# brendel-group/cl-ica

Hardware: AMD Instinct MI355X
Metric: training steps/sec (B=6144, n=10 MLP) (higher is better)
Workload: dtype f32 via f16x2 split (3 fp16 MFMA products of scaled two-piece operands, fp32 accumulate)

## Files before the change

cl_ica_amd/csrc/lp_finalize.h:

```cpp
#pragma once
#include "lp_kernels.h"

namespace clica {
namespace lp {

__device__ __forceinline__ float pos_sum(const float* a, const float* b, int n, const Params& q, bool frac) {
  float s = 0.f;
  for (int k = 0; k < n; ++k) {
    float d = a[k] - b[k];
    float t;
    if (frac) t = fexp2(q.p * flog2(fabsf(d) + 1e-12f));
    else if (q.p == 2.f) t = d * d;
    else if (q.p == 1.f) t = fabsf(d);
    else if (q.p == 3.f) t = fabsf(d) * d * d;
    else t = fabsf(d) > 0.f ? fexp2(q.p * flog2(fabsf(d))) : 0.f;
    s += t;
  }
  return s;
}


__device__ __forceinline__ float unfused(float t) { asm("" : "+v"(t)); return t; }
typedef const __attribute__((address_space(3))) float* lds_cfloat_ptr;
template <int W>
// ... 75 lines not shown
  const float sc = q.xs * C / tau;
  statC[i] = sc;
  if (statC_value) *statC_value = sc;
  if (!dz1 && !dz2) return;
  if (dot) {
    float pos = 0.f;
    if (q.posdot) pos = q.posdot[i];
    else for (int k = 0; k < q.n; ++k) pos += a[k] * b[k];
    const float dpos = -A / tau + (C / tau) * fexp2(pos * q.kscale - L2);
    if (q.dpos) { q.dpos[i] = dpos; return; }
    for (int k = 0; k < q.n; ++k) {
      if (dz1) dz1[i * ldd1 + k] = dpos * b[k];
      if (dz2) dz2[i * ldd2 + k] = dpos * a[k];
    }
    return;
  }
  const float sp_ = pos_sum(a, b, q.n, q, frac != 0);
  const float cpos = cpos_of(sp_, A, C, q, tau, compat, L2);
  for (int k = 0; k < q.n; ++k) {
    const float d = a[k] - b[k];
    float dt;
    if (frac) {
      const float v = fexp2((q.p - 1.f) * flog2(fabsf(d) + 1e-12f));
      dt = d > 0.f ? v : (d < 0.f ? -v : 0.f);
    } else if (q.p == 2.f) dt = d;
    else if (q.p == 1.f) dt = (d > 0.f ? 1.f : 0.f) - (d < 0.f ? 1.f : 0.f);
    else if (q.p == 3.f) dt = d * fabsf(d);
    else {
      const float ad = fabsf(d);
      const float v = ad > 0.f ? fexp2((q.p - 1.f) * flog2(ad)) : 0.f;
      dt = d < 0.f ? -v : v;
    }
    const float g = cpos * dt;
    if (dz1) dz1[i * ldd1 + k] = g;
    if (dz2) dz2[i * ldd2 + k] = -g;
  }
}

template <int W>
__device__ __forceinline__ void coef_row_regs(
    const int64_t i, const int64_t rows, const float (&a)[W], const float (&b)[W], const float sp_,
    const Params& q, float tau, float alpha, int compat, const float L2,
    float* __restrict__ statL, float* __restrict__ statC,
    float* __restrict__ dz1, int64_t ldd1, float* __restrict__ dz2, int64_t ldd2, float* statC_value) {
  const float inv_rows = 1.f / (float)rows;
  const float gi = 1.f * inv_rows + 0.f;
  const float A = 2.f * alpha * gi + 0.f;
  const float C = 2.f * (1.f - alpha) * gi + 0.f;
  statL[i] = L2;
  const float sc = q.xs * C / tau;
  statC[i] = sc;
  *statC_value = sc;
  if (!dz1 && !dz2) return;
  const float cpos = cpos_of(sp_, A, C, q, tau, compat, L2);
  const int n = q.n;
  auto put = [&](int k, float dt) {
    const float g = cpos * dt;
    if (k < n) {
      if (dz1) dz1[i * ldd1 + k] = g;
      if (dz2) dz2[i * ldd2 + k] = -g;
    }
  };
  if (q.p == 2.f) {
#pragma unroll
    for (int k = 0; k < W; ++k) { const float d = a[k] - b[k]; put(k, d); }
  } else if (q.p == 1.f) {
#pragma unroll
    for (int k = 0; k < W; ++k) { const float d = a[k] - b[k]; put(k, (d > 0.f ? 1.f : 0.f) - (d < 0.f ? 1.f : 0.f)); }
  } else if (q.p == 3.f) {
#pragma unroll
    for (int k = 0; k < W; ++k) { const float d = a[k] - b[k]; put(k, d * fabsf(d)); }
  } else {
#pragma unroll
    for (int k = 0; k < W; ++k) {
      const float d = a[k] - b[k];
      const float ad = fabsf(d);
      const float v = ad > 0.f ? fexp2((q.p - 1.f) * flog2(ad)) : 0.f;
      put(k, d < 0.f ? -v : v);
    }
  }
}


struct FinScratch { float* sm; float* ss; float* zr0; float* zr1; int zmaxn; float* ush; };
template <bool COHERENT = false, int W = 0>
__device__ __forceinline__ void finalize_rows(
    const int blk, const float2* __restrict__ part, const int nsplit, const int64_t rows,
    const float* __restrict__ z1, int64_t ld1, const float* __restrict__ z2, int64_t ld2,
    const Params& q, float tau, float alpha, int compat, int frac, int dot, float log_b3,
    float* __restrict__ loss_i, float* __restrict__ pos_i, float* __restrict__ lse_i, const TrainOut& T, const FinScratch& S,
    float& v_loss, float& v_pos, float& v_lse) {
  const int lane_row = threadIdx.x & (FIN_ROWS - 1), grp = threadIdx.x / FIN_ROWS;
  const int64_t i = (int64_t)blk * FIN_ROWS + lane_row;
  const bool staged = q.n <= S.zmaxn;
  if (staged) {
    const int64_t r0 = (int64_t)blk * FIN_ROWS;
    const int cnt = (int)min((int64_t)FIN_ROWS, rows - r0) * q.n;
    for (int idx = threadIdx.x; idx < cnt; idx += THREADS) {
      const int r = idx / q.n, k = idx - r * q.n;
      S.zr0[idx] = z1[(r0 + r) * ld1 + k];
      S.zr1[idx] = z2[(r0 + r) * ld2 + k];
    }
  }
  float m = -1e30f, s = 0.f;
  if (i < rows) {
    constexpr int G = THREADS / FIN_ROWS;
    for (int sp0 = grp; sp0 < nsplit; sp0 += 4 * G) {
      float2 ps[4];
#pragma unroll
      for (int u = 0; u < 4; ++u) {
        const int sp = sp0 + u * G;
        if (!(sp < nsplit)) ps[u] = make_float2(-1e30f, 0.f);
        else if (COHERENT)
          ps[u] = __builtin_bit_cast(float2, __hip_atomic_load(reinterpret_cast<const unsigned long long*>(part + (int64_t)sp * rows + i),
                                                                __ATOMIC_RELAXED, __HIP_MEMORY_SCOPE_AGENT));
        else ps[u] = part[(int64_t)sp * rows + i];
      }
#pragma unroll
      for (int u = 0; u < 4; ++u) {
        const float mn = fmaxf(m, ps[u].x);
        s = s * fexp2(m - mn) + ps[u].y * fexp2(ps[u].x - mn);
        m = mn;
      }
    }
  }
  S.sm[grp * FIN_ROWS + lane_row] = m; S.ss[grp * FIN_ROWS + lane_row] = s;
  __syncthreads();
  v_loss = 0.f; v_pos = 0.f; v_lse = 0.f;
  if (grp == 0 && i < rows) {
#pragma unroll
    for (int w = 1; w < THREADS / FIN_ROWS; ++w) {
      const float pm = S.sm[w * FIN_ROWS + lane_row], psum = S.ss[w * FIN_ROWS + lane_row];
      const float mn = fmaxf(m, pm);
      s = s * fexp2(m - mn) + psum * fexp2(pm - mn);
      m = mn;
    }
    float pos, xp;
    const float* ra = staged ? &S.zr0[lane_row * q.n] : z1 + i * ld1;
    const float* rb = staged ? &S.zr1[lane_row * q.n] : z2 + i * ld2;
    const bool regs = W > 0 && staged && !dot && !frac;
    float av[W > 0 ? W : 1], bv[W > 0 ? W : 1], sp_regs = 0.f;
    if constexpr (W > 0) {
      if (regs) { read_staged_row<W>(av, &S.zr0[lane_row * q.n], q.n); read_staged_row<W>(bv, &S.zr1[lane_row * q.n], q.n); }
    }
    if (dot) {
      pos = 0.f;
      if (q.posdot) pos = q.posdot[i];
      else for (int k = 0; k < q.n; ++k) pos += ra[k] * rb[k];
      xp = pos * q.kscale;
      pos = -pos;
    } else {
      float sp_;
      if constexpr (W > 0) sp_ = regs ? pos_sum_regs<W>(av, bv, q.n, q) : pos_sum(ra, rb, q.n, q, frac != 0);
      else sp_ = pos_sum(ra, rb, q.n, q, frac != 0);
      sp_regs = sp_;
      pos = q.pow ? sp_ : root_of<true>(sp_, q);
      xp = -pos * q.kscale;
    }
    if (compat) {
      const float mn = fmaxf(m, xp);
      s = s * fexp2(m - mn) + fexp2(xp - mn);
      m = mn;
    }
    const float L2 = m + flog2(s);
    const float lse_raw = L2 * kLn2;
    const float lse = compat ? lse_raw : lse_raw - log_b3;
    const float lp = pos / tau;
    const float li = 2.f * (alpha * lp + (1.f - alpha) * lse);
    loss_i[i] = li; pos_i[i] = lp; lse_i[i] = L2;
    float sc_i = 0.f;
    if (T.statL) {
      bool done = false;
      if constexpr (W > 0) {
        if (regs) { coef_row_regs<W>(i, rows, av, bv, sp_regs, q, tau, alpha, compat, L2, T.statL, T.statC, T.dz1, T.ldd1, T.dz2, T.ldd2, &sc_i); done = true; }
      }
      if (!done)
        coef_row(i, rows, ra, rb, q, tau, alpha, compat, frac, dot, L2, nullptr, nullptr, nullptr, nullptr, T.statL, T.statC,
                 T.dz1, T.ldd1, T.dz2, T.ldd2, &sc_i);
    }
    v_loss = li; v_pos = lp; v_lse = lse;
    if (S.ush) S.ush[lane_row] = sc_i * fexp2(-L2);
  } else if (S.ush && grp == 0) {
    S.ush[lane_row] = 0.f;
  }
}

struct FinArgs {
  const float* z2; int64_t ld2; float tau, alpha; int compat; float log_b3;
  float* loss_i; float* pos_i; float* lse_i; Means M; TrainOut T; int* arrive;
  float* means; float inv_count;
};
template <int NP, int PK, int R, bool ROOT, int NQ, bool ZMAX>
__global__ __launch_bounds__(THREADS, fwd_min_waves(NP, false)) void fwd_partial_fin_k(
    const float* __restrict__ own, int64_t ldo, int64_t n_own,
    const float* __restrict__ str, int64_t lds, int64_t n_str,
    Params q, float2* __restrict__ part, int chunk, FinArgs F) {
  static_assert(HALF * R == FIN_ROWS && NP <= 16, "an owner tile of the sweep = one finalize block; z rows staged in the tile buffers");
  float* scratch = nullptr;
  fwd_partial_body<NP, PK, R, ROOT, false, NQ, ZMAX>(own, ldo, n_own, str, lds, n_str, q, part, nullptr, chunk, blockIdx.x, blockIdx.y, &scratch);
  __shared__ float sm[THREADS / FIN_ROWS][FIN_ROWS], ss[THREADS / FIN_ROWS][FIN_ROWS];
  __shared__ int s_last;
  __builtin_amdgcn_s_waitcnt(0x0F70);
  __syncthreads();
  if (threadIdx.x == 0) {
    const int prev = __hip_atomic_fetch_add(&F.arrive[blockIdx.x], 1, __ATOMIC_RELAXED, __HIP_MEMORY_SCOPE_AGENT);
    s_last = prev == (int)gridDim.y - 1;
    if (s_last) __hip_atomic_store(&F.arrive[blockIdx.x], 0, __ATOMIC_RELAXED, __HIP_MEMORY_SCOPE_AGENT);
  }
  __syncthreads();
  LPT_STAMP(4);
  if (!s_last) { LPT_FLUSH(0); return; }
  float v_loss, v_pos, v_lse;
  constexpr int ZMAXN = 2 * tile_rows(NP) * NP / (2 * FIN_ROWS);
  static_assert(ZMAXN >= NP, "tile buffers too small for the z rows");
  finalize_rows<true, NP>((int)blockIdx.x, part, (int)gridDim.y, n_own, own, ldo, F.z2, F.ld2, q, F.tau, F.alpha, F.compat, 0, 0, F.log_b3,
                F.loss_i, F.pos_i, F.lse_i, F.T, FinScratch{&sm[0][0], &ss[0][0], scratch, scratch + FIN_ROWS * ZMAXN, ZMAXN, nullptr},
                v_loss, v_pos, v_lse);
  reduce_means(v_loss, v_pos, v_lse, F.M, (int)blockIdx.x, F.means != nullptr);
  LPT_STAMP(5);
  LPT_FLUSH(0);
  if (!F.means) return;
  __builtin_amdgcn_s_waitcnt(0x0F70);
  __syncthreads();
  if (threadIdx.x == 0) {
    const int prev = __hip_atomic_fetch_add(&F.arrive[gridDim.x], 1, __ATOMIC_RELAXED, __HIP_MEMORY_SCOPE_AGENT);
    s_last = prev == (int)gridDim.x - 1;
    if (s_last) __hip_atomic_store(&F.arrive[gridDim.x], 0, __ATOMIC_RELAXED, __HIP_MEMORY_SCOPE_AGENT);
  }
  __syncthreads();
  if (!s_last || threadIdx.x >= 64) return;
  float v[3] = {0.f, 0.f, 0.f};
  for (int b = threadIdx.x; b < (int)gridDim.x; b += 64) {
#pragma unroll
    for (int c = 0; c < 3; ++c) v[c] += __hip_atomic_load(&F.M.blocksums[b * 3 + c], __ATOMIC_RELAXED, __HIP_MEMORY_SCOPE_AGENT);
  }
#pragma unroll
  for (int a = 0; a < 3; ++a) {
#pragma unroll
    for (int off = 32; off > 0; off >>= 1) v[a] += __shfl_down(v[a], off, 64);
  }
  if (threadIdx.x == 0) { F.means[0] = v[0] * F.inv_count; F.means[1] = v[1] * F.inv_count; F.means[2] = v[2] * F.inv_count; }
}

#define CLICA_LP_DECLARE_FIN(PKV)                                                                          \
  bool launch_fwd_partial_fin_pk##PKV(const Plan& P, const float* own, int64_t ldo, int64_t n_own,        \
                                      const float* str, int64_t lds, int64_t n_str, const Params& q,      \
                                      float2* part, const FinArgs& F, hipStream_t st);
CLICA_LP_DECLARE_FIN(0) CLICA_LP_DECLARE_FIN(1) CLICA_LP_DECLARE_FIN(2) CLICA_LP_DECLARE_FIN(3) CLICA_LP_DECLARE_FIN(4)

}
}
```

cl_ica_amd/csrc/lp_kernels.h:

```cpp
#pragma once
#include "common.h"
#include <math.h>
#include <stdlib.h>
#include <type_traits>

namespace clica {
namespace lp {

constexpr int THREADS = 256;
constexpr int WAVES = THREADS / 64;
constexpr int HALF = 32;
constexpr int PARTS = 2 * WAVES;
constexpr int JB = 4;
#ifndef CLICA_LP_JBW
#define CLICA_LP_JBW 2
#endif
constexpr int jb_fwd(int np) { return np <= 16 ? 4 : 2; }
constexpr int JBW = CLICA_LP_JBW;
#ifndef CLICA_LP_TS16
#define CLICA_LP_TS16 128
#endif
#ifndef CLICA_LP_TS40
#define CLICA_LP_TS40 128
#endif
// ... 87 lines not shown
__device__ __forceinline__ float droot_of(float s, const Params& q) {
  if constexpr (!ROOT) return q.p;
  if (q.p == 1.f) return 1.f;
  return s > 0.f ? fexp2((q.inv_p - 1.f) * flog2(s)) : 0.f;
}

template <int NP>
struct Stager {
  static constexpr int TS = tile_rows(NP);
  static constexpr int ITERS = TS * NP / THREADS;
  static_assert((TS * NP) % THREADS == 0, "tile must divide over the workgroup");
  float v[ITERS];
  unsigned off[ITERS];
  bool kok[ITERS];
  const float* base;
  int64_t ld;
  int cnt;
  int nn;
  bool wide;
  __device__ __forceinline__ void init(const float* __restrict__ str, int64_t lds, int64_t j0, int n) {
    base = str + j0 * lds; ld = lds; cnt = 0; nn = n;
    wide = lds > (int64_t)(0x7fffffff / (4 * TS));
#pragma unroll
    for (int it = 0; it < ITERS; ++it) {
      const int idx = threadIdx.x + it * THREADS;
      const int row = idx / NP, k = idx - row * NP;
      kok[it] = k < n;
      off[it] = kok[it] ? ((unsigned)row * (unsigned)lds + (unsigned)k) * 4u : 0u;
    }
  }
  __device__ __forceinline__ void load(int c) {
    const char* b = reinterpret_cast<const char*>(base);
    cnt = c;
    if (!wide) {
      if (c == TS) {
#pragma unroll
        for (int it = 0; it < ITERS; ++it) v[it] = *reinterpret_cast<const float*>(b + off[it]);
      } else {
        const unsigned end = (unsigned)c * (unsigned)ld * 4u;
#pragma unroll
        for (int it = 0; it < ITERS; ++it) v[it] = *reinterpret_cast<const float*>(b + (off[it] < end ? off[it] : 0u));
      }
    }
    base += (int64_t)TS * ld;
  }
  __device__ __forceinline__ void store(float* tile, float pre = 1.f) const {
    if (wide) {
      const float* b = base - (int64_t)TS * ld;
#pragma unroll 1
      for (int idx = threadIdx.x; idx < TS * NP; idx += THREADS) {
        const int row = idx / NP, k = idx - row * NP;
        const bool ok = k < nn && row < cnt;
        const float x = b[ok ? (int64_t)row * ld + k : 0];
        tile[idx] = ok ? x * pre : 0.f;
      }
    } else if (cnt == TS) {
#pragma unroll
      for (int it = 0; it < ITERS; ++it) tile[threadIdx.x + it * THREADS] = kok[it] ? v[it] * pre : 0.f;
    } else {
      const unsigned end = (unsigned)cnt * (unsigned)ld * 4u;
#pragma unroll
      for (int it = 0; it < ITERS; ++it) tile[threadIdx.x + it * THREADS] = (kok[it] && off[it] < end) ? v[it] * pre : 0.f;
    }
  }
};

template <int NP, int R>
__device__ __forceinline__ void load_owners(f32x2 (&o)[R][NP / 2], const float* __restrict__ own, int64_t ldo,
                                            int64_t own0, int64_t n_own, int n, float pre = 1.f) {
  const int li = threadIdx.x & (HALF - 1);
#pragma unroll
  for (int r = 0; r < R; ++r) {
    const int64_t i = own0 + (int64_t)r * HALF + li;
    const bool ok = i < n_own;
#pragma unroll
    for (int k2 = 0; k2 < NP / 2; ++k2) {
      const bool a = ok && 2 * k2 < n, b = ok && 2 * k2 + 1 < n;
      const float x = own[a ? i * ldo + 2 * k2 : 0], y = own[b ? i * ldo + 2 * k2 + 1 : 0];
      o[r][k2].x = a ? x * pre : 0.f; o[r][k2].y = b ? y * pre : 0.f;
    }
  }
}

template <int NP, int PK, int NQ = NP / 2, int JBT = JB>
__device__ __forceinline__ void dist_group(const f32x2 (&o)[NP / 2], const float* tile, int jj, const Params& q,
                                           float (&acc)[JBT]) {
  f32x2 a2[JBT];
#pragma unroll
  for (int c = 0; c < JBT; ++c) a2[c] = (f32x2){0.f, 0.f};
#pragma unroll
  for (int k4 = 0; k4 < NP / 4; ++k4) {
#pragma unroll
    for (int c = 0; c < JBT; ++c) {
      const float4 sv = *reinterpret_cast<const float4*>(&tile[(jj + c) * NP + 4 * k4]);
      if (2 * k4 < NQ) accum2<PK>(a2[c], o[2 * k4], (f32x2){sv.x, sv.y}, q, 4 * k4);
      if (2 * k4 + 1 < NQ) accum2<PK>(a2[c], o[2 * k4 + 1], (f32x2){sv.z, sv.w}, q, 4 * k4 + 2);
    }
  }
#pragma unroll
  for (int c = 0; c < JBT; ++c) acc[c] = a2[c].x + a2[c].y;
}

template <int NP, int PK, int NQ = NP / 2, int JBT = JB>
__device__ __forceinline__ void dist_group_keep(const f32x2 (&o)[NP / 2], const float* tile, int jj, float (&acc)[JBT], f32x2 (&d)[JBT][NQ]) {
  static_assert(PK >= 1 && PK <= 3, "difference-based pair kinds");
  f32x2 a2[JBT];
#pragma unroll
  for (int c = 0; c < JBT; ++c) a2[c] = (f32x2){0.f, 0.f};
#pragma unroll
  for (int k4 = 0; k4 < NP / 4; ++k4) {
#pragma unroll
    for (int c = 0; c < JBT; ++c) {
      const float4 sv = *reinterpret_cast<const float4*>(&tile[(jj + c) * NP + 4 * k4]);
#pragma unroll
      for (int h2 = 0; h2 < 2; ++h2) {
        const int k2 = 2 * k4 + h2;
        if (k2 < NQ) {
          const f32x2 dd = o[k2] - (h2 ? (f32x2){sv.z, sv.w} : (f32x2){sv.x, sv.y});
          d[c][k2] = dd;
          if constexpr (PK == 2) a2[c] = __builtin_elementwise_fma(dd, dd, a2[c]);
          else if constexpr (PK == 1) { a2[c].x = add_abs(a2[c].x, dd.x); a2[c].y = add_abs(a2[c].y, dd.y); }
          else { const f32x2 t = dd * dd; a2[c].x = fmaf(fabsf(dd.x), t.x, a2[c].x); a2[c].y = fmaf(fabsf(dd.y), t.y, a2[c].y); }
        }
      }
    }
  }
#pragma unroll
  for (int c = 0; c < JBT; ++c) acc[c] = a2[c].x + a2[c].y;
}
template <int PK>
__device__ __forceinline__ void gaccum2_d(f32x2& g, float coef, f32x2 d) {
  const f32x2 c2 = {coef, coef};
  if constexpr (PK == 2) {
    g = __builtin_elementwise_fma(c2, d, g);
  } else if constexpr (PK == 1) {
    const f32x2 big = {0x1p126f, 0x1p126f};
    f32x2 t = d * big;
    t.x = __builtin_amdgcn_fmed3f(t.x, -1.f, 1.f); t.y = __builtin_amdgcn_fmed3f(t.y, -1.f, 1.f);
    g = __builtin_elementwise_fma(c2, t, g);
  } else {
    const f32x2 t = {d.x * fabsf(d.x), d.y * fabsf(d.y)};
    g = __builtin_elementwise_fma(c2, t, g);
  }
}

#ifdef CLICA_LP_TRACE
static __device__ unsigned long long* g_lp_trace = nullptr;
constexpr int LPT_MAXWG = 1024, LPT_MAXT = 8, LPT_HEAD = 8, LPT_NS = LPT_HEAD + 4 * LPT_MAXT;
__device__ __forceinline__ unsigned long long* lpt_buf() { __shared__ unsigned long long b[LPT_NS]; return b; }
#define LPT_INIT() do { if (threadIdx.x == 0) { for (int i_ = 0; i_ < LPT_NS; ++i_) lpt_buf()[i_] = 0; lpt_buf()[0] = __builtin_readcyclecounter(); } } while (0)
#define LPT_STAMP(slot) do { if (threadIdx.x == 0) lpt_buf()[slot] = __builtin_readcyclecounter(); } while (0)
#define LPT_TILE(t, ph) do { if (threadIdx.x == 0 && (t) < LPT_MAXT) lpt_buf()[LPT_HEAD + 4 * (t) + (ph)] = __builtin_readcyclecounter(); } while (0)
#define LPT_FLUSH(kind) do { if (threadIdx.x == 0 && g_lp_trace) { \
    const unsigned wg_ = blockIdx.y * gridDim.x + blockIdx.x; \
    lpt_buf()[6] = __builtin_readcyclecounter(); \
    if (wg_ < (unsigned)LPT_MAXWG) for (int i_ = 0; i_ < LPT_NS; ++i_) g_lp_trace[((size_t)(kind) * LPT_MAXWG + wg_) * LPT_NS + i_] = lpt_buf()[i_]; } } while (0)
#else
#define LPT_INIT() do { } while (0)
#define LPT_STAMP(slot) do { } while (0)
#define LPT_TILE(t, ph) do { } while (0)
#define LPT_FLUSH(kind) do { } while (0)
#endif

constexpr int fwd_min_waves(int np, bool rowgrad) { return rowgrad ? (np <= 16 ? 3 : 2) : (np <= 16 ? 4 : (np <= 24 ? 3 : 2)); }
constexpr int bwd_min_waves(int np) { return np <= 16 ? 3 : 2; }

template <int NP, int PK, int R, bool ROOT, bool ROWGRAD, int NQ = NP / 2, bool ZMAX = false>
__device__ __forceinline__ void fwd_partial_body(
    const float* __restrict__ own, int64_t ldo, int64_t n_own,
    const float* __restrict__ str, int64_t lds, int64_t n_str,
    const Params& q, float2* __restrict__ part, float* __restrict__ part_g, int chunk, const int bx, const int by,
    float** scratch_out = nullptr ) {
  constexpr int TS = tile_rows(NP), RPP = TS / PARTS, JBF = jb_fwd(NP);
  static_assert(RPP % JBF == 0, "partition rows must be whole JB groups");
  static_assert(WAVES * HALF * R * NP <= 2 * TS * NP, "the cross-wave merge reuses the tile buffers");
  __shared__ __attribute__((aligned(16))) float tiles[2][TS * NP];
  __shared__ float2 wred[WAVES][HALF * R];
  if (scratch_out) *scratch_out = &tiles[0][0];
  const int lane = threadIdx.x & 63, wave = threadIdx.x >> 6, li = lane & (HALF - 1), hf = lane >> 5;
  const int pq = wave * 2 + hf;
  const int64_t own0 = (int64_t)bx * (HALF * R);
  f32x2 o[R][NP / 2];
  f32x2 G[ROWGRAD ? R : 1][NP / 2];
  LPT_INIT();
  load_owners<NP, R>(o, own, ldo, own0, n_own, q.n, q.pre);
  LPT_STAMP(1);
  float m[R], s[R];
  const float csgn = (PK == 0) ? q.sgn : 1.f;
#pragma unroll
  for (int r = 0; r < (ROWGRAD ? R : 1); ++r)
#pragma unroll
    for (int k2 = 0; k2 < NP / 2; ++k2) G[r][k2] = (f32x2){0.f, 0.f};
  static_assert(!(ZMAX && ROWGRAD), "the fixed-maximum forward is the training sweep (no row gradient)");
#pragma unroll
  for (int r = 0; r < R; ++r) { m[r] = ZMAX ? 0.f : -INFINITY; s[r] = 0.f; }
  const float xk = q.xs * q.kscale;

  const int64_t jb = (int64_t)by * chunk;
  const int64_t je = min(n_str, jb + (int64_t)chunk);
  Stager<NP> st;
  if (jb < je) {
    st.init(str, lds, jb, q.n);
    st.load((int)min((int64_t)TS, je - jb));
    st.store(tiles[0], q.pre);
  }
  __syncthreads();
  LPT_STAMP(2);
  int cur = 0;
  for (int64_t j0 = jb; j0 < je; j0 += TS, cur ^= 1) {
    const int cnt = (int)min((int64_t)TS, je - j0);
    const bool more = j0 + TS < je;
    if (more) st.load((int)min((int64_t)TS, je - j0 - TS));
    LPT_TILE((int)((j0 - jb) / TS), 0);
    const float* tile = tiles[cur] + pq * RPP * NP;
    const int cq = min(RPP, max(0, cnt - pq * RPP));
    auto sweep = [&](auto ragged_tag) {
    constexpr bool RAGGED = decltype(ragged_tag)::value;
    for (int jj = 0; jj < cq; jj += JBF) {
#pragma unroll
      for (int r = 0; r < R; ++r) {
        float acc[JBF];
        dist_group<NP, PK, NQ, JBF>(o[r], tile, jj, q, acc);
        if constexpr (ZMAX) {
          float add = 0.f;
#pragma unroll
          for (int c = 0; c < JBF; ++c) add += (RAGGED && jj + c >= cq) ? 0.f : fexp2(PK == 1 ? acc[c] * xk : -acc[c]);
          s[r] += add;
          continue;
        }
        float x[JBF];
#pragma unroll
        for (int c = 0; c < JBF; ++c) {
          x[c] = root_of<ROOT>(acc[c], q) * xk;
          if (RAGGED && jj + c >= cq) x[c] = -INFINITY;
        }
        float xm = x[0];
#pragma unroll
        for (int c = 1; c < JBF; ++c) xm = fmaxf(xm, x[c]);
        const float mn = fmaxf(xm, fmaxf(m[r], -1e30f));
        float add = 0.f, e[JBF];
#pragma unroll
        for (int c = 0; c < JBF; ++c) { e[c] = fexp2(x[c] - mn); add += e[c]; }
        const float resc = fexp2(m[r] - mn);
        s[r] = fmaf(s[r], resc, add);
        m[r] = mn;
        if (ROWGRAD) {
#pragma unroll
          for (int c = 0; c < JBF; ++c) e[c] *= droot_of<ROOT>(acc[c], q) * csgn;
          asm volatile("" ::: "memory");
          const f32x2 r2 = {resc, resc};
#pragma unroll
          for (int k4 = 0; k4 < NP / 4; ++k4) {
            G[r][2 * k4] *= r2; G[r][2 * k4 + 1] *= r2;
#pragma unroll
            for (int c = 0; c < JBF; ++c) {
              const float4 sv = *reinterpret_cast<const float4*>(&tile[(jj + c) * NP + 4 * k4]);
              if (2 * k4 < NQ) gaccum2<PK>(G[r][2 * k4], e[c], o[r][2 * k4], (f32x2){sv.x, sv.y}, q, 4 * k4);
              if (2 * k4 + 1 < NQ) gaccum2<PK>(G[r][2 * k4 + 1], e[c], o[r][2 * k4 + 1], (f32x2){sv.z, sv.w}, q, 4 * k4 + 2);
            }
          }
        }
      }
    }
    };
    LPT_TILE((int)((j0 - jb) / TS), 1);
    if (cq == RPP) sweep(std::false_type{}); else sweep(std::true_type{});
    LPT_TILE((int)((j0 - jb) / TS), 2);
    if (more) st.store(tiles[cur ^ 1], q.pre);
    __syncthreads();
    LPT_TILE((int)((j0 - jb) / TS), 3);
  }
  float* gred = &tiles[0][0];
#pragma unroll
  for (int r = 0; r < R; ++r) {
    const float mo = __shfl_xor(m[r], HALF, 64), so = __shfl_xor(s[r], HALF, 64);
    const float mn = fmaxf(fmaxf(m[r], mo), -1e30f);
    const float fa = fexp2(m[r] - mn), fb = fexp2(mo - mn);
    const float s_lo = hf ? so : s[r], s_hi = hf ? s[r] : so, f_lo = hf ? fb : fa, f_hi = hf ? fa : fb;
    s[r] = fmaf(s_lo, f_lo, s_hi * f_hi);
    if (ROWGRAD) {
#pragma unroll
      for (int k2 = 0; k2 < NP / 2; ++k2) {
        const float gxo = __shfl_xor(G[r][k2].x, HALF, 64), gyo = __shfl_xor(G[r][k2].y, HALF, 64);
        const float gx_lo = hf ? gxo : G[r][k2].x, gx_hi = hf ? G[r][k2].x : gxo;
        const float gy_lo = hf ? gyo : G[r][k2].y, gy_hi = hf ? G[r][k2].y : gyo;
        G[r][k2].x = fmaf(gx_lo, f_lo, gx_hi * f_hi); G[r][k2].y = fmaf(gy_lo, f_lo, gy_hi * f_hi);
      }
    }
    m[r] = mn;
    if (hf == 0) {
      wred[wave][r * HALF + li] = make_float2(m[r], s[r]);
      if (ROWGRAD) {
        float4* dst = reinterpret_cast<float4*>(gred + ((size_t)wave * (HALF * R) + r * HALF + li) * NP);
#pragma unroll
        for (int k4 = 0; k4 < NP / 4; ++k4)
          dst[k4] = make_float4(G[r][2 * k4].x, G[r][2 * k4].y, G[r][2 * k4 + 1].x, G[r][2 * k4 + 1].y);
      }
    }
  }
  __syncthreads();
  if (threadIdx.x < HALF * R) {
    const int t = threadIdx.x;
    const int64_t i = own0 + t;
    float mm = -1e30f;
#pragma unroll
    for (int w = 0; w < WAVES; ++w) mm = fmaxf(mm, wred[w][t].x);
    float ss = 0.f, f[WAVES];
#pragma unroll
    for (int w = 0; w < WAVES; ++w) { f[w] = fexp2(wred[w][t].x - mm); ss = fmaf(wred[w][t].y, f[w], ss); }
    if (i < n_own) {
      if (scratch_out) {
        const float2 ms = make_float2(mm, ss);
        __hip_atomic_store(reinterpret_cast<unsigned long long*>(part + (int64_t)by * n_own + i), __builtin_bit_cast(unsigned long long, ms),
                           __ATOMIC_RELAXED, __HIP_MEMORY_SCOPE_AGENT);
      } else {
        part[(int64_t)by * n_own + i] = make_float2(mm, ss);
      }
      if (ROWGRAD) {
        float4* dst = reinterpret_cast<float4*>(part_g + ((int64_t)by * n_own + i) * NP);
#pragma unroll
        for (int k4 = 0; k4 < NP / 4; ++k4) {
          float4 a4 = make_float4(0.f, 0.f, 0.f, 0.f);
#pragma unroll
          for (int w = 0; w < WAVES; ++w) {
            const float4 g4 = *reinterpret_cast<const float4*>(gred + ((size_t)w * (HALF * R) + t) * NP + 4 * k4);
            a4.x = fmaf(g4.x, f[w], a4.x); a4.y = fmaf(g4.y, f[w], a4.y); a4.z = fmaf(g4.z, f[w], a4.z); a4.w = fmaf(g4.w, f[w], a4.w);
          }
          dst[k4] = a4;
        }
      }
    }
  }
  LPT_STAMP(3);
  if (!scratch_out) LPT_FLUSH(0);
}

template <int NP, int PK, int R, bool ROOT, bool ROWGRAD, int NQ = NP / 2, bool ZMAX = false>
__global__ __launch_bounds__(THREADS, fwd_min_waves(NP, ROWGRAD)) void fwd_partial_k(
    const float* __restrict__ own, int64_t ldo, int64_t n_own,
    const float* __restrict__ str, int64_t lds, int64_t n_str,
    Params q, float2* __restrict__ part, float* __restrict__ part_g, int chunk) {
  fwd_partial_body<NP, PK, R, ROOT, ROWGRAD, NQ, ZMAX>(own, ldo, n_own, str, lds, n_str, q, part, part_g, chunk, blockIdx.x, blockIdx.y);
}

template <int NP, int PK, int R, int STATS, bool ROOT, int NQ = NP / 2, bool FOLD = false>
__device__ __forceinline__ void bwd_pairs_body(
    const float* __restrict__ own, int64_t ldo, int64_t n_own,
    const float* __restrict__ str, int64_t lds, int64_t n_str,
    const Params& q, const float* __restrict__ statL, const float* __restrict__ statC,
    const float* __restrict__ strL, const float* __restrict__ strC,
    float* __restrict__ part, int chunk, const int bx, const int by) {
  constexpr bool OWNER_STATS = (STATS & 1) != 0, STREAM_STATS = (STATS & 2) != 0;
  constexpr int TS = tile_rows(NP), RPP = TS / PARTS;
  static_assert(WAVES * HALF * R * NP <= 2 * TS * NP, "the cross-wave merge reuses the tile buffers");
  __shared__ __attribute__((aligned(16))) float tiles[2][TS * NP];
  __shared__ float tLs[2][TS], tCs[2][TS];
  const int lane = threadIdx.x & 63, wave = threadIdx.x >> 6, li = lane & (HALF - 1), hf = lane >> 5;
  const int pq = wave * 2 + hf;
  const int64_t own0 = (int64_t)bx * (HALF * R);
  f32x2 o[R][NP / 2], g[R][NP / 2];
  LPT_INIT();
  load_owners<NP, R>(o, own, ldo, own0, n_own, q.n, q.pre);
  LPT_STAMP(1);
  float oL[R], oC[R];
#pragma unroll
  for (int r = 0; r < R; ++r) {
    const int64_t i = own0 + (int64_t)r * HALF + li;
    oL[r] = 0.f; oC[r] = 0.f;
    if (OWNER_STATS && i < n_own) { oL[r] = statL[i]; oC[r] = statC[i]; }
    if (FOLD) oC[r] *= fexp2(-oL[r]) * q.gfold;
#pragma unroll
    for (int k2 = 0; k2 < NP / 2; ++k2) g[r][k2] = (f32x2){0.f, 0.f};
  }
  const float xk = q.xs * q.kscale;
  const float csgn = (PK == 0) ? q.sgn : 1.f;
  const int64_t jb = (int64_t)by * chunk;
  const int64_t je = min(n_str, jb + (int64_t)chunk);
  Stager<NP> st;
  float rl = 0.f, rc = 0.f;
  auto load_stats = [&](int64_t j0, int cnt) {
    if (STREAM_STATS && (int)threadIdx.x < TS) {
      const bool ok = (int)threadIdx.x < cnt;
      rl = strL[ok ? j0 + threadIdx.x : 0]; rc = strC[ok ? j0 + threadIdx.x : 0];
    }
  };
  auto store_stats = [&](int b) {
    if (STREAM_STATS && (int)threadIdx.x < TS) {
      const bool ok = (int)threadIdx.x < st.cnt;
      const float l = ok ? rl : 0.f, c = ok ? rc : 0.f;
      tLs[b][threadIdx.x] = l; tCs[b][threadIdx.x] = FOLD ? c * fexp2(-l) * q.gfold : c;
    }
  };
  if (jb < je) {
    const int c0 = (int)min((int64_t)TS, je - jb);
    st.init(str, lds, jb, q.n);
    st.load(c0); load_stats(jb, c0);
    st.store(tiles[0], q.pre); store_stats(0);
  }
  __syncthreads();
  LPT_STAMP(2);
  int cur = 0;
  for (int64_t j0 = jb; j0 < je; j0 += TS, cur ^= 1) {
    const int cnt = (int)min((int64_t)TS, je - j0);
    const bool more = j0 + TS < je;
    if (more) {
      const int c1 = (int)min((int64_t)TS, je - j0 - TS);
      st.load(c1); load_stats(j0 + TS, c1);
    }
    LPT_TILE((int)((j0 - jb) / TS), 0);
    const float* tile = tiles[cur] + pq * RPP * NP;
    const float* tL = tLs[cur] + pq * RPP;
    const float* tC = tCs[cur] + pq * RPP;
    const int cq = min(RPP, max(0, cnt - pq * RPP));
#ifndef CLICA_LP_KEEPD_WIDE
#define CLICA_LP_KEEPD_WIDE 1
#endif
    constexpr bool KEEPD = PK >= 1 && PK <= 3 && (NP <= 16 || (CLICA_LP_KEEPD_WIDE && NP <= 40));
    constexpr int JW = KEEPD ? 1 : JBW;
    LPT_TILE((int)((j0 - jb) / TS), 1);
    for (int jj = 0; jj < cq; jj += JW) {
#pragma unroll
      for (int r = 0; r < R; ++r) {
        float acc[JW];
        f32x2 dk[JW][KEEPD ? NQ : 1];
        if constexpr (KEEPD) dist_group_keep<NP, PK, NQ, JW>(o[r], tile, jj, acc, dk);
        else dist_group<NP, PK, NQ, JW>(o[r], tile, jj, q, acc);
        float coef[JW];
#pragma unroll
        for (int c = 0; c < JW; ++c) {
          if constexpr (FOLD) {
            static_assert(!FOLD || (STATS == 3 && !ROOT), "folded coefficient: symmetric training sweep only");
            float cf = fexp2(PK == 1 ? acc[c] * xk : -acc[c]) * (oC[r] + tC[jj + c]);
            if (jj + c >= cq) cf = 0.f;
            coef[c] = cf;
            continue;
          }
          const float x = root_of<ROOT>(acc[c], q) * xk;
          float w = 0.f;
          if constexpr (FOLD) {
          } else {
            if (OWNER_STATS) w = oC[r] * fexp2(x - oL[r]);
            if (STREAM_STATS) w = fmaf(tC[jj + c], fexp2(x - tL[jj + c]), w);
          }
          float cf = w * droot_of<ROOT>(acc[c], q) * csgn;
          if (OWNER_STATS && jj + c >= cq) cf = 0.f;
          coef[c] = cf;
        }
        if constexpr (KEEPD) {
#pragma unroll
          for (int k2 = 0; k2 < NQ; ++k2)
#pragma unroll
            for (int c = 0; c < JW; ++c) gaccum2_d<PK>(g[r][k2], coef[c], dk[c][k2]);
        } else {
          asm volatile("" ::: "memory");
#pragma unroll
          for (int k4 = 0; k4 < NP / 4; ++k4) {
#pragma unroll
            for (int c = 0; c < JW; ++c) {
              const float4 sv = *reinterpret_cast<const float4*>(&tile[(jj + c) * NP + 4 * k4]);
              if (2 * k4 < NQ) gaccum2<PK>(g[r][2 * k4], coef[c], o[r][2 * k4], (f32x2){sv.x, sv.y}, q, 4 * k4);
              if (2 * k4 + 1 < NQ) gaccum2<PK>(g[r][2 * k4 + 1], coef[c], o[r][2 * k4 + 1], (f32x2){sv.z, sv.w}, q, 4 * k4 + 2);
            }
          }
        }
      }
    }
    LPT_TILE((int)((j0 - jb) / TS), 2);
    if (more) { st.store(tiles[cur ^ 1], q.pre); store_stats(cur ^ 1); }
    __syncthreads();
    LPT_TILE((int)((j0 - jb) / TS), 3);
  }
  float* gred = &tiles[0][0];
#pragma unroll
  for (int r = 0; r < R; ++r) {
#pragma unroll
    for (int k2 = 0; k2 < NP / 2; ++k2) {
      const float gxo = __shfl_xor(g[r][k2].x, HALF, 64), gyo = __shfl_xor(g[r][k2].y, HALF, 64);
      g[r][k2].x = hf ? gxo + g[r][k2].x : g[r][k2].x + gxo;
      g[r][k2].y = hf ? gyo + g[r][k2].y : g[r][k2].y + gyo;
    }
    if (hf == 0) {
      float4* dst = reinterpret_cast<float4*>(gred + ((size_t)wave * (HALF * R) + r * HALF + li) * NP);
#pragma unroll
      for (int k4 = 0; k4 < NP / 4; ++k4)
        dst[k4] = make_float4(g[r][2 * k4].x, g[r][2 * k4].y, g[r][2 * k4 + 1].x, g[r][2 * k4 + 1].y);
    }
  }
  __syncthreads();
  constexpr int Q4 = NP / 4;
  for (int u = threadIdx.x; u < HALF * R * Q4; u += THREADS) {
    const int t = u / Q4, k4 = u - t * Q4;
    const int64_t i = own0 + t;
    if (i >= n_own) continue;
    float4 a4 = *reinterpret_cast<const float4*>(gred + (size_t)t * NP + 4 * k4);
#pragma unroll
    for (int w = 1; w < WAVES; ++w) {
      const float4 g4 = *reinterpret_cast<const float4*>(gred + ((size_t)w * (HALF * R) + t) * NP + 4 * k4);
      a4.x += g4.x; a4.y += g4.y; a4.z += g4.z; a4.w += g4.w;
    }
    *reinterpret_cast<float4*>(part + ((int64_t)by * n_own + i) * NP + 4 * k4) = a4;
  }
  LPT_STAMP(3);
  LPT_FLUSH(1);
}

template <int NP, int PK, int R, int STATS, bool ROOT, int NQ = NP / 2, bool FOLD = false>
__global__ __launch_bounds__(THREADS, bwd_min_waves(NP)) void bwd_pairs_k(
    const float* __restrict__ own, int64_t ldo, int64_t n_own,
    const float* __restrict__ str, int64_t lds, int64_t n_str,
    Params q, const float* __restrict__ statL, const float* __restrict__ statC,
    const float* __restrict__ strL, const float* __restrict__ strC,
    float* __restrict__ part, int chunk) {
  bwd_pairs_body<NP, PK, R, STATS, ROOT, NQ, FOLD>(own, ldo, n_own, str, lds, n_str, q, statL, statC, strL, strC, part, chunk, blockIdx.x, blockIdx.y);
}

constexpr int W_OWN = 16, W_KL = 16;
constexpr int kMaxWideN = 512;
constexpr int wide_kc(int n) { return n <= 128 ? 8 : (n <= 256 ? 16 : 32); }
constexpr int wide_ts(int kc) { return kc == 32 ? 16 : 32; }
enum WideMode { W_FWD = 0, W_FWD_ROWGRAD = 1, W_BWD_OWNER = 2, W_BWD_STREAM = 3, W_BWD_SYM = 4 };

template <int PK>
__device__ __forceinline__ float term1(float o, float s, const Params& q) {
  if constexpr (PK == PK_DOT) return o * s;
  else if constexpr (PK == 2) { const float d = o - s; return d * d; }
  else if constexpr (PK == 1) return fabsf(o - s);
  else if constexpr (PK == 3) { const float d = o - s; return fabsf(d) * d * d; }
  else { const float a = fabsf(q.sgn * (o - s) + q.eps); return a > 0.f ? fexp2(q.p * flog2(a)) : 0.f; }
}
template <int PK>
__device__ __forceinline__ float dterm1(float o, float s, const Params& q) {
  if constexpr (PK == PK_DOT) return s;
  else if constexpr (PK == 2) return o - s;
  else if constexpr (PK == 1) { const float d = o - s; return d > 0.f ? 1.f : (d < 0.f ? -1.f : 0.f); }
  else if constexpr (PK == 3) { const float d = o - s; return d * fabsf(d); }
  else {
    const float e = q.sgn * (o - s) + q.eps, a = fabsf(e);
    const float v = a > 0.f ? fexp2((q.p - 1.f) * flog2(a)) : 0.f;
    return e < 0.f ? -v : v;
  }
}

template <int KC, int PK, int MODE>
__global__ __launch_bounds__(THREADS) void wide_k(
    const float* __restrict__ own, int64_t ldo, int64_t n_own,
    const float* __restrict__ str, int64_t lds, int64_t n_str, Params q,
    const float* __restrict__ ownL, const float* __restrict__ ownC,
    const float* __restrict__ strL, const float* __restrict__ strC,
    float2* __restrict__ part, float* __restrict__ part_g, int np, int chunk) {
  constexpr bool FWD = MODE == W_FWD || MODE == W_FWD_ROWGRAD, ROWGRAD = MODE == W_FWD_ROWGRAD;
  constexpr bool OWNER_STATS = MODE == W_BWD_OWNER || MODE == W_BWD_SYM, STREAM_STATS = MODE == W_BWD_STREAM || MODE == W_BWD_SYM;
  constexpr bool GRAD = MODE != W_FWD;
  constexpr int TS = wide_ts(KC), LDT = KC * W_KL;
  __shared__ __attribute__((aligned(16))) float tile[TS * LDT];
  __shared__ float tL[TS], tC[TS];
  const int oi = threadIdx.x >> 4, kl = threadIdx.x & (W_KL - 1);
  const int64_t i = (int64_t)blockIdx.x * W_OWN + oi;
  const bool own_ok = i < n_own;
  float o[KC], g[GRAD ? KC : 1];
#pragma unroll
  for (int c = 0; c < KC; ++c) {
    const int k = kl + W_KL * c;
    const bool ok = own_ok && k < q.n;
    const float x = own[ok ? i * ldo + k : 0];
    o[c] = ok ? x : 0.f;
  }
#pragma unroll
  for (int c = 0; c < (GRAD ? KC : 1); ++c) g[c] = 0.f;
  float oL = 0.f, oC = 0.f;
  if (OWNER_STATS && own_ok) { oL = ownL[i]; oC = ownC[i]; }
  float m = -INFINITY, s = 0.f;
  const float xk = q.xs * q.kscale;
  const float csgn = (PK == 0) ? q.sgn : 1.f;
  const bool root = !q.pow;
  const int64_t jb = (int64_t)blockIdx.y * chunk;
  const int64_t je = min(n_str, jb + (int64_t)chunk);
  for (int64_t j0 = jb; j0 < je; j0 += TS) {
    const int cnt = (int)min((int64_t)TS, je - j0);
    __syncthreads();
    for (int idx = threadIdx.x; idx < TS * LDT; idx += THREADS) {
      const int row = idx / LDT, k = idx - row * LDT;
      const bool ok = row < cnt && k < q.n;
      const float x = str[ok ? (j0 + row) * lds + k : 0];
      tile[idx] = ok ? x : 0.f;
    }
    if (STREAM_STATS && (int)threadIdx.x < TS) {
      const bool ok = (int)threadIdx.x < cnt;
      const float l = strL[ok ? j0 + threadIdx.x : 0], c = strC[ok ? j0 + threadIdx.x : 0];
      tL[threadIdx.x] = ok ? l : 0.f; tC[threadIdx.x] = ok ? c : 0.f;
    }
    __syncthreads();
    for (int jj = 0; jj < cnt; ++jj) {
      const float* row = tile + jj * LDT + kl;
      float acc = 0.f;
#pragma unroll
// ... 137 lines not shown
```

Baseline: 2712.

## Stage owner and partner rows through LDS with coalesced loads in pair kernels

Owner rows in the forward and backward pair kernels are now loaded with a flat, coalesced per-thread pattern into dedicated shared buffers and then read back as float4 into registers, in place of per-lane strided loads. The fused finalize kernel also prefetches the partner (z2) rows at the start, so the finalize step reads both rows from these shared buffers instead of re-gathering them into the tile buffers afterward. Kernel arguments are pinned into scalar registers with empty asm to force early s_load. This adds LDS per block, which could lower occupancy, and adds an extra barrier-bound copy through LDS.

```diff
diff --git a/cl_ica_amd/csrc/lp_finalize.h b/cl_ica_amd/csrc/lp_finalize.h
--- a/cl_ica_amd/csrc/lp_finalize.h
+++ b/cl_ica_amd/csrc/lp_finalize.h
@@ -181,7 +181,7 @@
 }
 
 
-struct FinScratch { float* sm; float* ss; float* zr0; float* zr1; int zmaxn; float* ush; };
+struct FinScratch { float* sm; float* ss; const float* zr0; const float* zr1; int zmaxn; float* ush; int zld = 0; };
 template <bool COHERENT = false, int W = 0>
 __device__ __forceinline__ void finalize_rows(
     const int blk, const float2* __restrict__ part, const int nsplit, const int64_t rows,
@@ -192,13 +192,15 @@
   const int lane_row = threadIdx.x & (FIN_ROWS - 1), grp = threadIdx.x / FIN_ROWS;
   const int64_t i = (int64_t)blk * FIN_ROWS + lane_row;
   const bool staged = q.n <= S.zmaxn;
-  if (staged) {
+  const int zld = S.zld > 0 ? S.zld : q.n;
+  if (staged && S.zld == 0) {
+    float* w0 = const_cast<float*>(S.zr0); float* w1 = const_cast<float*>(S.zr1);
     const int64_t r0 = (int64_t)blk * FIN_ROWS;
     const int cnt = (int)min((int64_t)FIN_ROWS, rows - r0) * q.n;
     for (int idx = threadIdx.x; idx < cnt; idx += THREADS) {
       const int r = idx / q.n, k = idx - r * q.n;
-      S.zr0[idx] = z1[(r0 + r) * ld1 + k];
-      S.zr1[idx] = z2[(r0 + r) * ld2 + k];
+      w0[idx] = z1[(r0 + r) * ld1 + k];
+      w1[idx] = z2[(r0 + r) * ld2 + k];
     }
   }
   float m = -1e30f, s = 0.f;
@@ -235,12 +237,12 @@
       m = mn;
     }
     float pos, xp;
-    const float* ra = staged ? &S.zr0[lane_row * q.n] : z1 + i * ld1;
-    const float* rb = staged ? &S.zr1[lane_row * q.n] : z2 + i * ld2;
+    const float* ra = staged ? &S.zr0[lane_row * zld] : z1 + i * ld1;
+    const float* rb = staged ? &S.zr1[lane_row * zld] : z2 + i * ld2;
     const bool regs = W > 0 && staged && !dot && !frac;
     float av[W > 0 ? W : 1], bv[W > 0 ? W : 1], sp_regs = 0.f;
     if constexpr (W > 0) {
-      if (regs) { read_staged_row<W>(av, &S.zr0[lane_row * q.n], q.n); read_staged_row<W>(bv, &S.zr1[lane_row * q.n], q.n); }
+      if (regs) { read_staged_row<W>(av, ra, q.n); read_staged_row<W>(bv, rb, q.n); }
     }
     if (dot) {
       pos = 0.f;
@@ -294,26 +296,31 @@
     const float* __restrict__ own, int64_t ldo, int64_t n_own,
     const float* __restrict__ str, int64_t lds, int64_t n_str,
     Params q, float2* __restrict__ part, int chunk, FinArgs F) {
-  static_assert(HALF * R == FIN_ROWS && NP <= 16, "an owner tile of the sweep = one finalize block; z rows staged in the tile buffers");
-  float* scratch = nullptr;
-  fwd_partial_body<NP, PK, R, ROOT, false, NQ, ZMAX>(own, ldo, n_own, str, lds, n_str, q, part, nullptr, chunk, blockIdx.x, blockIdx.y, &scratch);
+  static_assert(HALF * R == FIN_ROWS && NP <= 16, "an owner tile of the sweep = one finalize block; rows of at most 16 coordinates in registers");
+  LP_PIN_HEAD_ARGS();
+  asm volatile("" :: "s"(part), "s"(F.z2), "s"(F.ld2), "s"(F.tau), "s"(F.alpha), "s"(F.compat), "s"(F.log_b3), "s"(F.loss_i), "s"(F.pos_i), "s"(F.lse_i),
+               "s"(F.M.blocksums), "s"(F.T.statL), "s"(F.T.statC), "s"(F.T.dz1), "s"(F.T.ldd1), "s"(F.T.dz2), "s"(F.T.ldd2), "s"(F.arrive),
+               "s"(F.means), "s"(F.inv_count));
+  FinStage fin;
+  fin.z2 = F.z2; fin.ld2 = F.ld2;
+  fwd_partial_body<NP, PK, R, ROOT, false, NQ, ZMAX, true>(own, ldo, n_own, str, lds, n_str, q, part, nullptr, chunk, blockIdx.x, blockIdx.y, &fin);
   __shared__ float sm[THREADS / FIN_ROWS][FIN_ROWS], ss[THREADS / FIN_ROWS][FIN_ROWS];
   __shared__ int s_last;
+  const int nsplit = (int)gridDim.y;
+  asm volatile("" :: "s"(nsplit));
   __builtin_amdgcn_s_waitcnt(0x0F70);
   __syncthreads();
   if (threadIdx.x == 0) {
     const int prev = __hip_atomic_fetch_add(&F.arrive[blockIdx.x], 1, __ATOMIC_RELAXED, __HIP_MEMORY_SCOPE_AGENT);
-    s_last = prev == (int)gridDim.y - 1;
+    s_last = prev == nsplit - 1;
     if (s_last) __hip_atomic_store(&F.arrive[blockIdx.x], 0, __ATOMIC_RELAXED, __HIP_MEMORY_SCOPE_AGENT);
   }
   __syncthreads();
   LPT_STAMP(4);
   if (!s_last) { LPT_FLUSH(0); return; }
   float v_loss, v_pos, v_lse;
-  constexpr int ZMAXN = 2 * tile_rows(NP) * NP / (2 * FIN_ROWS);
-  static_assert(ZMAXN >= NP, "tile buffers too small for the z rows");
-  finalize_rows<true, NP>((int)blockIdx.x, part, (int)gridDim.y, n_own, own, ldo, F.z2, F.ld2, q, F.tau, F.alpha, F.compat, 0, 0, F.log_b3,
-                F.loss_i, F.pos_i, F.lse_i, F.T, FinScratch{&sm[0][0], &ss[0][0], scratch, scratch + FIN_ROWS * ZMAXN, ZMAXN, nullptr},
+  finalize_rows<true, NP>((int)blockIdx.x, part, nsplit, n_own, own, ldo, F.z2, F.ld2, q, F.tau, F.alpha, F.compat, 0, 0, F.log_b3,
+                F.loss_i, F.pos_i, F.lse_i, F.T, FinScratch{&sm[0][0], &ss[0][0], fin.owners, fin.partners, NP, nullptr, NP},
                 v_loss, v_pos, v_lse);
   reduce_means(v_loss, v_pos, v_lse, F.M, (int)blockIdx.x, F.means != nullptr);
   LPT_STAMP(5);
diff --git a/cl_ica_amd/csrc/lp_kernels.h b/cl_ica_amd/csrc/lp_kernels.h
--- a/cl_ica_amd/csrc/lp_kernels.h
+++ b/cl_ica_amd/csrc/lp_kernels.h
@@ -193,6 +193,59 @@
   }
 }
 
+template <int NP, int R>
+struct OwnerStager {
+  static constexpr int ROWS = HALF * R, ITERS = ROWS * NP / THREADS;
+  static_assert((ROWS * NP) % THREADS == 0, "owner tile must divide over the workgroup");
+  float v[ITERS];
+  __device__ __forceinline__ void load(const float* __restrict__ own, int64_t ldo, int64_t own0, int64_t n_own, int n) {
+    const bool any = own0 < n_own;
+    const float* base = own + (any ? own0 : 0) * ldo;
+    const int cnt = any ? (int)min((int64_t)ROWS, n_own - own0) : 0;
+    const bool wide = ldo > (int64_t)(0x7fffffff / (4 * ROWS));
+    if (!wide) {
+      const char* b = reinterpret_cast<const char*>(base);
+#pragma unroll
+      for (int it = 0; it < ITERS; ++it) {
+        const int idx = threadIdx.x + it * THREADS;
+        const int row = idx / NP, k = idx - row * NP;
+        const unsigned off = (k < n && row < cnt) ? ((unsigned)row * (unsigned)ldo + (unsigned)k) * 4u : 0u;
+        v[it] = *reinterpret_cast<const float*>(b + off);
+      }
+    } else {
+#pragma unroll
+      for (int it = 0; it < ITERS; ++it) {
+        const int idx = threadIdx.x + it * THREADS;
+        const int row = idx / NP, k = idx - row * NP;
+        v[it] = base[(k < n && row < cnt) ? (int64_t)row * ldo + k : 0];
+      }
+    }
+  }
+  __device__ __forceinline__ void store(float* area) const {
+#pragma unroll
+    for (int it = 0; it < ITERS; ++it) area[threadIdx.x + it * THREADS] = v[it];
+  }
+  static __device__ __forceinline__ void read(f32x2 (&o)[R][NP / 2], const float* area, int64_t own0, int64_t n_own, int n, float pre) {
+    const int li = threadIdx.x & (HALF - 1);
+#pragma unroll
+    for (int r = 0; r < R; ++r) {
+      const bool rok = own0 + (int64_t)r * HALF + li < n_own;
+      const float4* src = reinterpret_cast<const float4*>(area + (r * HALF + li) * NP);
+#pragma unroll
+      for (int k4 = 0; k4 < NP / 4; ++k4) {
+        const float4 x = src[k4];
+        o[r][2 * k4].x = (rok && 4 * k4 < n) ? x.x * pre : 0.f; o[r][2 * k4].y = (rok && 4 * k4 + 1 < n) ? x.y * pre : 0.f;
+        o[r][2 * k4 + 1].x = (rok && 4 * k4 + 2 < n) ? x.z * pre : 0.f; o[r][2 * k4 + 1].y = (rok && 4 * k4 + 3 < n) ? x.w * pre : 0.f;
+      }
+    }
+  }
+};
+struct FinStage {
+  const float* z2; int64_t ld2;
+  const float* owners;
+  const float* partners;
+};
+
 template <int NP, int PK, int NQ = NP / 2, int JBT = JB>
 __device__ __forceinline__ void dist_group(const f32x2 (&o)[NP / 2], const float* tile, int jj, const Params& q,
                                            float (&acc)[JBT]) {
@@ -273,28 +326,35 @@
 #define LPT_FLUSH(kind) do { } while (0)
 #endif
 
+#define LP_PIN_HEAD_ARGS() \
+  asm volatile("" :: "s"(own), "s"(ldo), "s"(n_own), "s"(str), "s"(lds), "s"(n_str), "s"(q.n), "s"(q.pre), "s"(chunk))
+
 constexpr int fwd_min_waves(int np, bool rowgrad) { return rowgrad ? (np <= 16 ? 3 : 2) : (np <= 16 ? 4 : (np <= 24 ? 3 : 2)); }
 constexpr int bwd_min_waves(int np) { return np <= 16 ? 3 : 2; }
 
-template <int NP, int PK, int R, bool ROOT, bool ROWGRAD, int NQ = NP / 2, bool ZMAX = false>
+template <int NP, int PK, int R, bool ROOT, bool ROWGRAD, int NQ = NP / 2, bool ZMAX = false, bool FIN = false>
 __device__ __forceinline__ void fwd_partial_body(
     const float* __restrict__ own, int64_t ldo, int64_t n_own,
     const float* __restrict__ str, int64_t lds, int64_t n_str,
     const Params& q, float2* __restrict__ part, float* __restrict__ part_g, int chunk, const int bx, const int by,
-    float** scratch_out = nullptr ) {
+    FinStage* fin = nullptr ) {
   constexpr int TS = tile_rows(NP), RPP = TS / PARTS, JBF = jb_fwd(NP);
   static_assert(RPP % JBF == 0, "partition rows must be whole JB groups");
   static_assert(WAVES * HALF * R * NP <= 2 * TS * NP, "the cross-wave merge reuses the tile buffers");
   __shared__ __attribute__((aligned(16))) float tiles[2][TS * NP];
   __shared__ float2 wred[WAVES][HALF * R];
-  if (scratch_out) *scratch_out = &tiles[0][0];
+  __shared__ __attribute__((aligned(16))) float owners[HALF * R * NP];
+  __shared__ __attribute__((aligned(16))) float partners[FIN ? HALF * R * NP : 4];
+  if constexpr (FIN) { fin->owners = owners; fin->partners = partners; }
   const int lane = threadIdx.x & 63, wave = threadIdx.x >> 6, li = lane & (HALF - 1), hf = lane >> 5;
   const int pq = wave * 2 + hf;
   const int64_t own0 = (int64_t)bx * (HALF * R);
   f32x2 o[R][NP / 2];
   f32x2 G[ROWGRAD ? R : 1][NP / 2];
   LPT_INIT();
-  load_owners<NP, R>(o, own, ldo, own0, n_own, q.n, q.pre);
+  OwnerStager<NP, R> ost, zst;
+  ost.load(own, ldo, own0, n_own, q.n);
+  if constexpr (FIN) zst.load(fin->z2, fin->ld2, own0, n_own, q.n);
   LPT_STAMP(1);
   float m[R], s[R];
   const float csgn = (PK == 0) ? q.sgn : 1.f;
@@ -313,9 +373,12 @@
   if (jb < je) {
     st.init(str, lds, jb, q.n);
     st.load((int)min((int64_t)TS, je - jb));
-    st.store(tiles[0], q.pre);
-  }
+  }
+  ost.store(owners);
+  if constexpr (FIN) zst.store(partners);
+  if (jb < je) st.store(tiles[0], q.pre);
   __syncthreads();
+  OwnerStager<NP, R>::read(o, owners, own0, n_own, q.n, q.pre);
   LPT_STAMP(2);
   int cur = 0;
   for (int64_t j0 = jb; j0 < je; j0 += TS, cur ^= 1) {
@@ -420,7 +483,7 @@
 #pragma unroll
     for (int w = 0; w < WAVES; ++w) { f[w] = fexp2(wred[w][t].x - mm); ss = fmaf(wred[w][t].y, f[w], ss); }
     if (i < n_own) {
-      if (scratch_out) {
+      if constexpr (FIN) {
         const float2 ms = make_float2(mm, ss);
         __hip_atomic_store(reinterpret_cast<unsigned long long*>(part + (int64_t)by * n_own + i), __builtin_bit_cast(unsigned long long, ms),
                            __ATOMIC_RELAXED, __HIP_MEMORY_SCOPE_AGENT);
@@ -443,7 +506,7 @@
     }
   }
   LPT_STAMP(3);
-  if (!scratch_out) LPT_FLUSH(0);
+  if constexpr (!FIN) LPT_FLUSH(0);
 }
 
 template <int NP, int PK, int R, bool ROOT, bool ROWGRAD, int NQ = NP / 2, bool ZMAX = false>
@@ -451,6 +514,7 @@
     const float* __restrict__ own, int64_t ldo, int64_t n_own,
     const float* __restrict__ str, int64_t lds, int64_t n_str,
     Params q, float2* __restrict__ part, float* __restrict__ part_g, int chunk) {
+  LP_PIN_HEAD_ARGS();
   fwd_partial_body<NP, PK, R, ROOT, ROWGRAD, NQ, ZMAX>(own, ldo, n_own, str, lds, n_str, q, part, part_g, chunk, blockIdx.x, blockIdx.y);
 }
 
@@ -466,23 +530,23 @@
   static_assert(WAVES * HALF * R * NP <= 2 * TS * NP, "the cross-wave merge reuses the tile buffers");
   __shared__ __attribute__((aligned(16))) float tiles[2][TS * NP];
   __shared__ float tLs[2][TS], tCs[2][TS];
+  __shared__ __attribute__((aligned(16))) float owners[HALF * R * NP];
+  __shared__ float oLs[HALF * R], oCs[HALF * R];
   const int lane = threadIdx.x & 63, wave = threadIdx.x >> 6, li = lane & (HALF - 1), hf = lane >> 5;
   const int pq = wave * 2 + hf;
   const int64_t own0 = (int64_t)bx * (HALF * R);
   f32x2 o[R][NP / 2], g[R][NP / 2];
   LPT_INIT();
-  load_owners<NP, R>(o, own, ldo, own0, n_own, q.n, q.pre);
+  OwnerStager<NP, R> ost;
+  ost.load(own, ldo, own0, n_own, q.n);
+  float osl = 0.f, osc = 0.f;
+  const bool os_ok = OWNER_STATS && (int)threadIdx.x < HALF * R && own0 + threadIdx.x < n_own;
+  if (OWNER_STATS && (int)threadIdx.x < HALF * R) { osl = statL[os_ok ? own0 + threadIdx.x : 0]; osc = statC[os_ok ? own0 + threadIdx.x : 0]; }
+  auto store_owners = [&]() {
+    ost.store(owners);
+    if ((int)threadIdx.x < HALF * R) { oLs[threadIdx.x] = os_ok ? osl : 0.f; oCs[threadIdx.x] = os_ok ? osc : 0.f; }
+  };
   LPT_STAMP(1);
-  float oL[R], oC[R];
-#pragma unroll
-  for (int r = 0; r < R; ++r) {
-    const int64_t i = own0 + (int64_t)r * HALF + li;
-    oL[r] = 0.f; oC[r] = 0.f;
-    if (OWNER_STATS && i < n_own) { oL[r] = statL[i]; oC[r] = statC[i]; }
-    if (FOLD) oC[r] *= fexp2(-oL[r]) * q.gfold;
-#pragma unroll
-    for (int k2 = 0; k2 < NP / 2; ++k2) g[r][k2] = (f32x2){0.f, 0.f};
-  }
   const float xk = q.xs * q.kscale;
   const float csgn = (PK == 0) ? q.sgn : 1.f;
   const int64_t jb = (int64_t)by * chunk;
@@ -506,9 +570,21 @@
     const int c0 = (int)min((int64_t)TS, je - jb);
     st.init(str, lds, jb, q.n);
     st.load(c0); load_stats(jb, c0);
+    store_owners();
     st.store(tiles[0], q.pre); store_stats(0);
+  } else {
+    store_owners();
   }
   __syncthreads();
+  OwnerStager<NP, R>::read(o, owners, own0, n_own, q.n, q.pre);
+  float oL[R], oC[R];
+#pragma unroll
+  for (int r = 0; r < R; ++r) {
+    oL[r] = oLs[r * HALF + li]; oC[r] = oCs[r * HALF + li];
+    if (FOLD) oC[r] *= fexp2(-oL[r]) * q.gfold;
+#pragma unroll
+    for (int k2 = 0; k2 < NP / 2; ++k2) g[r][k2] = (f32x2){0.f, 0.f};
+  }
   LPT_STAMP(2);
   int cur = 0;
   for (int64_t j0 = jb; j0 < je; j0 += TS, cur ^= 1) {
@@ -622,6 +698,8 @@
     Params q, const float* __restrict__ statL, const float* __restrict__ statC,
     const float* __restrict__ strL, const float* __restrict__ strC,
     float* __restrict__ part, int chunk) {
+  LP_PIN_HEAD_ARGS();
+  asm volatile("" :: "s"(statL), "s"(statC), "s"(strL), "s"(strC), "s"(q.gfold));
   bwd_pairs_body<NP, PK, R, STATS, ROOT, NQ, FOLD>(own, ldo, n_own, str, lds, n_str, q, statL, statC, strL, strC, part, chunk, blockIdx.x, blockIdx.y);
 }
 
```

Result: no change. 2696 (-0.6%).
